# nintendops/DynamicFusion_Body

Measured on AMD Instinct MI355X. Metric: Mvoxels/s TSDF fusion + GN-iters/s warp solve, 256³ grid, 1/2/4/8 GPU, higher is better.
Workload: dtype f64 geometry / f32 volume

## Files before the change

### dynamicfusion_body_amd/csrc/dfh_common.h

```cpp
#pragma once
#include <hip/hip_runtime.h>

#include <cstdarg>
#include <cstdio>

#include "../../include/dfusion_hip.h"

namespace dfh {

char *last_error_buf();
int fail(int code, const char *fmt, ...);

#define DFH_HIP_CHECK(expr)                                                               \
    do {                                                                                  \
        hipError_t _e = (expr);                                                           \
        if (_e != hipSuccess)                                                             \
            return ::dfh::fail(DFH_E_HIP, "%s failed: %s", #expr, hipGetErrorString(_e)); \
    } while (0)

#define DFH_REQUIRE(cond, ...)                                  \
    do {                                                        \
        if (!(cond)) return ::dfh::fail(DFH_E_BADARG, __VA_ARGS__); \
    } while (0)

inline int check_slab(const char *what, const dfh_slab *s) {
    DFH_REQUIRE(s, "%s: null slab", what);
    DFH_REQUIRE(s->res[0] > 0 && s->res[1] > 0 && s->res[2] > 0, "%s: bad grid %dx%dx%d", what, s->res[0], s->res[1], s->res[2]);
    DFH_REQUIRE(0 <= s->x0 && s->x0 <= s->x1 && s->x1 <= s->res[0], "%s: slab [%d,%d) outside [0,%d)", what, s->x0, s->x1, s->res[0]);
    DFH_REQUIRE(s->x1 - s->x0 <= 65535, "%s: slab has more than 65535 planes", what);
    return DFH_OK;
}

inline int check_volume(const char *what, const dfh_volume *v) {
    DFH_REQUIRE(v && v->tsdf && v->tsdf_w, "%s: null volume", what);
    DFH_REQUIRE(v->dtype == DFH_F32 || v->dtype == DFH_F64, "%s: bad volume dtype %d", what, v->dtype);
    return check_slab(what, &v->slab);
}

struct Mat3 { double m[9]; };
struct Mat34 { double m[12]; };
struct Vec3 { double v[3]; };
struct DQ { double q[8]; };

constexpr int kWave = 64;
#ifndef DFH_GN_TILE
#define DFH_GN_TILE 128
#endif
constexpr int kGnTile = DFH_GN_TILE;

#define DFH_OPTION_LIST(X)                                                                                                \
    X(k1_strided) X(k1_late_loads) X(k1_planes_per_block) X(k1_force_scalar) X(k1_bricks_min) X(k1_no_bricks)            \
    X(k1_bricks_nocull) X(k1_no_multi) X(k1_cull) X(k1_nzi) X(k1_prefetch) X(k1_nt) X(k1_gather_first)                  \
    X(k2_exact) X(k2_no_strided) X(k2_nt) X(k3_no_cache) X(k3_exact) X(k3_no_lds) X(k3_wg_per_cu) X(k3_tpb) X(k3_skip) X(plan_radix) X(rigid_atomic) X(gn_reg_own_launch) X(gn_reg_own_gather) \
    X(dbg_gather_part) X(pcg_wpb) X(pcg_multilaunch) X(pcg_spin_limit) X(pcg_one_xcd) X(gn_iter_own_clear) X(gn_gather_full) X(gn_no_view_cull)                                                            \
    X(py_plan_torch) X(py_allreduce_full) X(py_gn_atomic) X(py_gn_no_fused_assoc) X(py_gn_no_fused_iter) X(py_gn_iter_per_call) X(py_no_side_stream) X(py_no_host_scalars)
struct Options {
#define DFH_X(n) long n;
    DFH_OPTION_LIST(DFH_X)
#undef DFH_X
};
const Options &opt();

struct DeviceInfo {
    int n_cu = 0;
    int pcg_occ512 = -1, pcg_occ1024 = -1;
};
DeviceInfo &device_info(int device);
inline bool on(long v) { return v > 0; }

}
```

### dynamicfusion_body_amd/csrc/dfh_plan.hip

```cpp
#include "dfh_common.h"

#include <cstring>

#include <rocprim/device/device_radix_sort.hpp>

namespace dfh {

#ifndef DFH_SORT_BLOCK_ITEMS
#define DFH_SORT_BLOCK_ITEMS 8
#endif
using SortCfg = rocprim::radix_sort_config<rocprim::default_config,
                                           rocprim::merge_sort_config<512, 512, DFH_SORT_BLOCK_ITEMS, 128, 256, 8>,
                                           rocprim::default_config>;
constexpr int kPlanTile = kGnTile;
constexpr int kPlanWaves = kPlanTile / 64;
constexpr int kKMaxP = 8;

__device__ __forceinline__ int plan_find_block(const int *__restrict__ row_ptr, const int *__restrict__ col, int a, int b) {
    int lo = row_ptr[a], hi = row_ptr[a + 1] - 1;
    while (lo <= hi) {
        const int mid = (lo + hi) >> 1;
        const int c = col[mid];
        if (c == b) return mid;
        if (c < b) lo = mid + 1; else hi = mid - 1;
    }
    return -1;
}

__global__ __launch_bounds__(256) void plan_pack_keys_kernel(const int *__restrict__ nbr, int S, int k, unsigned long long N,
                                                              unsigned long long *__restrict__ key, int *__restrict__ idx) {
    const int s = blockIdx.x * 256 + threadIdx.x;
    if (s >= S) return;
    unsigned long long kk = 0;
    for (int j = 0; j < k; ++j) kk = kk * N + (unsigned long long)nbr[(size_t)s * k + j];
    key[s] = kk;
    idx[s] = s;
}

__global__ __launch_bounds__(256) void plan_permute_kernel(const int *__restrict__ order, int S, int k, const double *__restrict__ pos,
                                                           const double *__restrict__ nrm, const int *__restrict__ nbr,
                                                           const double *__restrict__ wts, double *__restrict__ pos_o,
                                                           double *__restrict__ nrm_o, int *__restrict__ nbr_o, double *__restrict__ wts_o) {
    const int i = blockIdx.x * 256 + threadIdx.x;
    if (i >= S) return;
    const size_t src = (size_t)order[i];
#pragma unroll
    for (int c = 0; c < 3; ++c) {
        pos_o[3 * (size_t)i + c] = pos[3 * src + c];
        nrm_o[3 * (size_t)i + c] = nrm[3 * src + c];
    }
    for (int j = 0; j < k; ++j) {
        nbr_o[(size_t)i * k + j] = nbr[src * k + j];
        wts_o[(size_t)i * k + j] = wts[src * k + j];
    }
}

__device__ __forceinline__ bool plan_is_head(const int *__restrict__ nbr, int s, int k) {
    if ((s & (kPlanTile - 1)) == 0) return true;
    bool h = false;
    for (int j = 0; j < k; ++j) h = h || nbr[(size_t)s * k + j] != nbr[(size_t)(s - 1) * k + j];
    return h;
}

__global__ __launch_bounds__(kPlanTile) void plan_heads_kernel(const int *__restrict__ nbr, int S, int k, int *__restrict__ tile_rows) {
    __shared__ int cnt[kPlanWaves];
    const int s = blockIdx.x * kPlanTile + threadIdx.x;
    const bool head = s < S && plan_is_head(nbr, s, k);
    const unsigned long long b = __ballot(head);
    if ((threadIdx.x & 63) == 0) cnt[threadIdx.x >> 6] = __popcll(b);
    __syncthreads();
    if (threadIdx.x == 0) {
        int n = 0;
        for (int w = 0; w < kPlanWaves; ++w) n += cnt[w];
        tile_rows[blockIdx.x] = n;
    }
}

__global__ __launch_bounds__(1024) void plan_scan_kernel(int *__restrict__ tile_rows, int n_tiles, int *__restrict__ n_rows_out) {
    __shared__ int wsum[16];
    __shared__ int carry_s;
    const int lane = threadIdx.x & 63, wv = threadIdx.x >> 6;
    if (threadIdx.x == 0) carry_s = 0;
    __syncthreads();
    for (int base = 0; base < n_tiles; base += 1024) {
        const int i = base + threadIdx.x;
        const int v = i < n_tiles ? tile_rows[i] : 0;
        int x = v;
#pragma unroll
        for (int o = 1; o < 64; o <<= 1) {
            const int y = __shfl_up(x, o, 64);
            if (lane >= o) x += y;
        }
        if (lane == 63) wsum[wv] = x;
        __syncthreads();
        int off = carry_s;
        for (int w = 0; w < wv; ++w) off += wsum[w];
        if (i < n_tiles) tile_rows[i] = off + x - v;
        __syncthreads();
        if (threadIdx.x == 1023) carry_s = off + x;
        __syncthreads();
    }
    if (threadIdx.x == 0) { tile_rows[n_tiles] = carry_s; *n_rows_out = carry_s; }
}

__global__ __launch_bounds__(kPlanTile) void plan_runid_kernel(const int *__restrict__ nbr, int S, int k, const int *__restrict__ tile_off,
                                                          int *__restrict__ run_id, int *__restrict__ row_first) {
    __shared__ int cnt[kPlanWaves];
    const int s = blockIdx.x * kPlanTile + threadIdx.x;
    const int lane = threadIdx.x & 63, wv = threadIdx.x >> 6;
    const bool head = s < S && plan_is_head(nbr, s, k);
    const unsigned long long b = __ballot(head);
    if (lane == 0) cnt[wv] = __popcll(b);
    __syncthreads();
    int r = tile_off[blockIdx.x] + __popcll(b & ((2ull << lane) - 1ull)) - 1;
    for (int w = 0; w < wv; ++w) r += cnt[w];
    if (s < S) {
        run_id[s] = r;
        if (head) row_first[r] = s;
    }
}

__device__ __forceinline__ int plan_count_slot(int *__restrict__ cnt, int key, bool active) {
    const int lane = threadIdx.x & 63;
    unsigned long long todo = __ballot(active);
    int leader = lane, rank = 0, size = 0;
    while (todo) {
        const int l0 = __ffsll((long long)todo) - 1;
        const int k0 = __shfl(key, l0, 64);
        const unsigned long long same = __ballot(active && key == k0) & todo;
        if (active && key == k0) {
            leader = l0;
            rank = __popcll(same & ((1ull << lane) - 1ull));
            size = __popcll(same);
        }
        todo &= ~same;
    }
    int base = 0;
    if (active && leader == lane) base = atomicAdd(cnt + key, size);
    base = __shfl(base, leader, 64);
    return base + rank;
}

__global__ __launch_bounds__(256) void plan_keys_kernel(const int *__restrict__ nbr, const int *__restrict__ row_first, int n_rows, int k,
                                                         const int *__restrict__ row_ptr, const int *__restrict__ col, int B,
                                                         int *__restrict__ blk_key, int *__restrict__ blk_val, int *__restrict__ node_key,
                                                         int *__restrict__ node_val, int *__restrict__ uncovered,
                                                         int *__restrict__ blk_cnt, int *__restrict__ node_cnt) {
    const int row = blockIdx.x * 256 + threadIdx.x;
    const int pr = blockIdx.y, kk = k * k;
    const int sa = pr / k, sb = pr - sa * k;
    const bool in = row < n_rows;
    int blk = B, nb = 0;
    if (in) {
        const size_t s0 = (size_t)row_first[row] * k;
        const int na = nbr[s0 + sa];
        nb = nbr[s0 + sb];
        blk = plan_find_block(row_ptr, col, na, nb);
        if (blk < 0) { blk = B; atomicOr(uncovered, 1); }
    }
    const int slot = plan_count_slot(blk_cnt, blk, in && blk < B);
    if (in) {
        const size_t e = (size_t)row * kk + pr;
        blk_key[e] = blk;
        blk_val[e] = blk < B ? slot : 0;
    }
    if (sa == 0) {
        const int nslot = plan_count_slot(node_cnt, nb, in);
        if (in) {
            node_key[(size_t)row * k + sb] = nb;
            node_val[(size_t)row * k + sb] = nslot;
        }
    }
}

__global__ __launch_bounds__(256) void plan_zero2_kernel(int *__restrict__ a, int na, int *__restrict__ b, int nb) {
    const int i = blockIdx.x * 256 + threadIdx.x;
    if (i < na) a[i] = 0;
    else if (i - na < nb) b[i - na] = 0;
}

__global__ void plan_flag_out_kernel(const int *__restrict__ flag_in, int *__restrict__ flag_out) { *flag_out = *flag_in; }

__global__ __launch_bounds__(1024) void plan_scan2_kernel(int *__restrict__ a, int na, int *__restrict__ b, int nb,
                                                           const int *__restrict__ flag_in, int *__restrict__ flag_out) {
    __shared__ int wsum[16];
    __shared__ int carry_s;
    if (blockIdx.x == 0 && threadIdx.x == 0) *flag_out = *flag_in;
    int *v_ = blockIdx.x == 0 ? a : b;
    const int n = blockIdx.x == 0 ? na : nb;
    const int lane = threadIdx.x & 63, wv = threadIdx.x >> 6;
    if (threadIdx.x == 0) carry_s = 0;
    __syncthreads();
    constexpr int C = 16;
    for (int base = 0; base < n; base += 1024 * C) {
        const int per = min(C, (min(n - base, 1024 * C) + 1023) / 1024);
        const int i0 = base + (int)threadIdx.x * per;
        int v[C];
        int sum = 0;
#pragma unroll
        for (int j = 0; j < C; ++j) {
            v[j] = (j < per && i0 + j < n) ? v_[i0 + j] : 0;
            sum += v[j];
        }
        int x = sum;
#pragma unroll
        for (int o = 1; o < 64; o <<= 1) {
            const int y = __shfl_up(x, o, 64);
            if (lane >= o) x += y;
        }
        if (lane == 63) wsum[wv] = x;
        __syncthreads();
        int off = carry_s;
        for (int w = 0; w < wv; ++w) off += wsum[w];
        int run = off + x - sum;
#pragma unroll
        for (int j = 0; j < C; ++j) {
            if (j < per && i0 + j < n) v_[i0 + j] = run;
            run += v[j];
        }
        __syncthreads();
        if (threadIdx.x == 1023) carry_s = off + x;
        __syncthreads();
    }
    if (threadIdx.x == 0) v_[n] = carry_s;
}

__global__ __launch_bounds__(256) void plan_fill_kernel(const int *__restrict__ blk_key, const int *__restrict__ blk_rank, long E, int B,
                                                         const int *__restrict__ blk_ptr, int *__restrict__ blk_ent,
                                                         const int *__restrict__ node_key, const int *__restrict__ node_rank, long E2,
                                                         const int *__restrict__ node_ptr, int *__restrict__ node_ent) {
    const long e = (long)blockIdx.x * 256 + threadIdx.x;
    if (e < E) {
        const int blk = blk_key[e];
        if (blk < B) blk_ent[blk_ptr[blk] + blk_rank[e]] = (int)e;
    }
    if (e < E2) node_ent[node_ptr[node_key[e]] + node_rank[e]] = (int)e;
}

constexpr int kListLds = 2048;
// ... 217 lines not shown
```

### dynamicfusion_body_amd/csrc/dfh_solve.hip

```cpp
#include "dfh_dq.h"

#include <algorithm>
#include <cmath>
#include <cstring>

namespace dfh {

constexpr int kKMaxS = 8;

struct Q4 { double w, x, y, z; };

__device__ __forceinline__ Q4 qmul(const Q4 &a, const Q4 &b) {
    Q4 o;
    o.w = a.w * b.w - a.x * b.x - a.y * b.y - a.z * b.z;
    o.x = a.w * b.x + a.x * b.w + a.y * b.z - a.z * b.y;
    o.y = a.w * b.y - a.x * b.z + a.y * b.w + a.z * b.x;
    o.z = a.w * b.z + a.x * b.y - a.y * b.x + a.z * b.w;
    return o;
}
__device__ __forceinline__ Q4 qconj(const Q4 &a) { return Q4{a.w, -a.x, -a.y, -a.z}; }
__device__ __forceinline__ Q4 qpure(double x, double y, double z) { return Q4{0.0, x, y, z}; }
__device__ __forceinline__ Q4 qadd(const Q4 &a, const Q4 &b) { return Q4{a.w + b.w, a.x + b.x, a.y + b.y, a.z + b.z}; }
__device__ __forceinline__ Q4 qscale(const Q4 &a, double s) { return Q4{a.w * s, a.x * s, a.y * s, a.z * s}; }

// ... 807 lines not shown
    if (ASSOC && aa.views && aa.cull) {
        __shared__ double sBox[kTileWaves][6];
        __shared__ unsigned sMask;
        const bool in = tid < tile_n;
        double bx[6] = {in ? a_xp.x : __builtin_huge_val(), in ? -a_xp.x : __builtin_huge_val(), in ? a_xp.y : __builtin_huge_val(),
                        in ? -a_xp.y : __builtin_huge_val(), in ? a_xp.z : __builtin_huge_val(), in ? -a_xp.z : __builtin_huge_val()};
#pragma unroll
        for (int o = 32; o > 0; o >>= 1)
#pragma unroll
            for (int c6 = 0; c6 < 6; ++c6) bx[c6] = fmin(bx[c6], __shfl_xor(bx[c6], o, 64));
        if ((tid & 63) == 0)
#pragma unroll
            for (int c6 = 0; c6 < 6; ++c6) sBox[tid >> 6][c6] = bx[c6];
        __syncthreads();
        double box[6];
#pragma unroll
        for (int c6 = 0; c6 < 6; ++c6) {
            double m = sBox[0][c6];
#pragma unroll
            for (int w_ = 1; w_ < kTileWaves; ++w_) m = fmin(m, sBox[w_][c6]);
            box[c6] = (c6 & 1) ? -m : m;
        }
        view_mask = tile_view_mask(aa.ap, aa.views, aa.n_views, box, &sMask);
    }
    if (ASSOC && tid < tile_n)
        a_ok = associate_views<float>(aa.ap, aa.views, aa.n_views, a_xp, a_c, view_mask);
    auto store_assoc = [&]() {
        if (ASSOC && tid < tile_n) {
            corr[3 * (size_t)s] = a_c[0]; corr[3 * (size_t)s + 1] = a_c[1]; corr[3 * (size_t)s + 2] = a_c[2];
            valid[s] = a_ok ? 1 : 0;
        }
    };
    const bool act = ASSOC ? a_ok : (tid < tile_n && valid[s] != 0);
    BT_STAMP(1);
    __shared__ int sWaveCnt[kTileWaves];
    const unsigned long long bal = __ballot(act);
    const int lane = tid & 63, wv = tid >> 6;
    if (lane == 0) sWaveCnt[wv] = __popcll(bal);
    __syncthreads();
    int pos = __popcll(bal & ((1ull << lane) - 1ull));
    for (int w_ = 0; w_ < wv; ++w_) pos += sWaveCnt[w_];
    int n_valid = 0;
#pragma unroll
    for (int w_ = 0; w_ < kTileWaves; ++w_) n_valid += sWaveCnt[w_];
    constexpr int ST_ = gn_row_stride(K);
    double *live = PLANNED ? tile_cost + 2 * (size_t)rt.n_tiles : nullptr;
    const int row_first = PLANNED ? run_id[blockIdx.x * kTile] : 0;
    const int rows_tile = PLANNED ? run_id[blockIdx.x * kTile + tile_n - 1] - row_first + 1 : 0;
    if (n_valid == 0) {
        store_assoc();
        if (PLANNED && tid < rows_tile) live[row_first + tid] = 0.0;
        if (PLANNED && tid == 0) { tile_cost[2 * blockIdx.x] = 0.0; tile_cost[2 * blockIdx.x + 1] = 0.0; }
        return;
    }
    if (!PLANNED && tid == 0) atomicAdd(cost_count + 1, (double)n_valid);
    __shared__ unsigned short sRow[PLANNED ? kTile : 1];
    __shared__ double sObj[kTileWaves];
    double obj = 0.0;
    if (act) {
        if (PLANNED) sRow[pos] = (unsigned short)(run_id[s] - row_first);
        double Jrow[NJ];
        double r;
        if (ASSOC) {
            r = data_row_from(node_dq, idx, w, K, p.lw.q, a_bh, a_nb, a_pf[0], a_pf[1], a_pf[2], a_xp, a_n[0], a_n[1], a_n[2], a_c[0], a_c[1],
                              a_c[2], Jrow);
        } else {
#pragma unroll
            for (int j = 0; j < kKMaxS; ++j) {
                idx[j] = j < K ? nbr[(size_t)s * K + j] : 0;
                w[j] = j < K ? wts[(size_t)s * K + j] : 0.0;
            }
            r = data_row(node_dq, idx, w, K, p.lw.q, spos[3 * (size_t)s], spos[3 * (size_t)s + 1], spos[3 * (size_t)s + 2],
                         snrm[3 * (size_t)s], snrm[3 * (size_t)s + 1], snrm[3 * (size_t)s + 2], corr[3 * (size_t)s],
                         corr[3 * (size_t)s + 1], corr[3 * (size_t)s + 2], Jrow);
        }
        obj = 0.5 * r * r;
        if (p.huber > 0.0 && fabs(r) > p.huber) {
            obj = p.huber * (fabs(r) - 0.5 * p.huber);
            const double sc = sqrt(p.huber / fabs(r));
            r *= sc;
#pragma unroll
            for (int j = 0; j < NJ; ++j) Jrow[j] *= sc;
        }
        if (!PLANNED) {
#pragma unroll
            for (int j = 0; j < K; ++j) sIdx[pos * K + j] = idx[j];
        }
#pragma unroll
        for (int j = 0; j < NJ; ++j) sJ[pos * LD + j] = Jrow[j];
        sJ[pos * LD + NJ] = r;
    }
    store_assoc();
    BT_STAMP(2);
    if (PLANNED) {
#pragma unroll
        for (int o = 32; o > 0; o >>= 1) obj += __shfl_xor(obj, o, 64);
        if (lane == 0) sObj[wv] = obj;
    }
    __syncthreads();
    if (PLANNED && tid == 0) {
        double o = sObj[0];
#pragma unroll
        for (int w_ = 1; w_ < kTileWaves; ++w_) o += sObj[w_];
        tile_cost[2 * blockIdx.x] = o;
        tile_cost[2 * blockIdx.x + 1] = (double)n_valid;
    }
    __shared__ int sRun[kTile + 1];
    __shared__ int sNRuns;
    {
        bool head = false;
        if (tid < n_valid) {
            head = tid == 0;
            if (!head) {
                if (PLANNED) {
                    head = sRow[tid] != sRow[tid - 1];
                } else {
#pragma unroll
                    for (int j = 0; j < K; ++j) head = head || (sIdx[tid * K + j] != sIdx[(tid - 1) * K + j]);
                }
            }
        }
        const unsigned long long hb = __ballot(head);
        if (lane == 0) sWaveCnt[wv] = __popcll(hb);
        __syncthreads();
        int hp = __popcll(hb & ((1ull << lane) - 1ull));
        for (int w_ = 0; w_ < wv; ++w_) hp += sWaveCnt[w_];
        if (head) sRun[hp] = tid;
        if (tid == 0) {
            int n = 0;
            for (int w_ = 0; w_ < kTileWaves; ++w_) n += sWaveCnt[w_];
            sRun[n] = n_valid;
            sNRuns = n;
        }
        __syncthreads();
    }
    const int n_runs = sNRuns;
    BT_STAMP(3);
#ifdef DFH_BUILD_TRACE
    if (threadIdx.x == 0 && blockIdx.x < 8192) g_build_trace[blockIdx.x][6] = (unsigned long long)n_valid | ((unsigned long long)n_runs << 16);
#endif
    constexpr bool kBlkTable = K <= 4 && !PLANNED;
    __shared__ int sBlk[kBlkTable ? kTile * K * K : 1];
    if (kBlkTable) {
        for (int q = tid; q < n_runs * K * K; q += kTile) {
            const int rn = q / (K * K), pr = q - rn * (K * K);
            const int t0 = sRun[rn];
            sBlk[q] = find_block(row_ptr, col, sIdx[t0 * K + pr / K], sIdx[t0 * K + pr % K]);
        }
        __syncthreads();
    }
    constexpr int NUP = PLANNED ? gn_row_gram(K) : NJ * (NJ + 1) / 2;
    if (PLANNED) {
        if (tid < n_runs) partial[(size_t)(row_first + sRow[sRun[tid]]) * ST_ + NUP + NJ + 1] = (double)(sRun[tid + 1] - sRun[tid]);
        __shared__ int sTouched[kTile];
        if (tid < rows_tile) sTouched[tid] = 0;
        __syncthreads();
        if (tid < n_runs) sTouched[sRow[sRun[tid]]] = 1;
        __syncthreads();
        if (tid < rows_tile) live[row_first + tid] = sTouched[tid] ? 1.0 : 0.0;
    }
    BT_STAMP(4);
    if constexpr (PLANNED) {
        constexpr int NC = NJ + 1;
        constexpr int NT = (NC + 15) / 16;
        typedef double d4 __attribute__((ext_vector_type(4)));
        const int li = lane & 15, lk = lane >> 4;
        for (int rn = wv; rn < n_runs; rn += kTile / 64) {
            const int t0 = sRun[rn], t1 = sRun[rn + 1];
            d4 acc[NT * (NT + 1) / 2];
#pragma unroll
            for (int q = 0; q < NT * (NT + 1) / 2; ++q) acc[q] = d4{0.0, 0.0, 0.0, 0.0};
            for (int t = t0; t < t1; t += 4) {
// ... 2237 lines not shown
```

### dynamicfusion_body_amd/solve.py

```python

import ctypes

import numpy as np
import torch

from . import _lib, dist as _dist
from .device import HostScalar, current_stream_ptr, dtype_code, require_gpu


def _f64(a, shape_tail=None):
    t = a if isinstance(a, torch.Tensor) else torch.from_numpy(np.ascontiguousarray(np.asarray(a, dtype=np.float64)))
    t = t.to(device="cuda", dtype=torch.float64).contiguous()
    if shape_tail is not None and tuple(t.shape[1:]) != tuple(shape_tail):
        raise ValueError("array has shape %s, expected (n,%s)" % (tuple(t.shape), ",".join(map(str, shape_tail))))
    return t


def _i32(a, shape_tail=None):
    t = a if isinstance(a, torch.Tensor) else torch.from_numpy(np.ascontiguousarray(np.asarray(a)))
    t = t.to(device="cuda", dtype=torch.int32).contiguous()
    if shape_tail is not None and tuple(t.shape[1:]) != tuple(shape_tail):
        raise ValueError("index array has shape %s, expected (n,%s)" % (tuple(t.shape), ",".join(map(str, shape_tail))))
    return t

# ... 145 lines not shown

    def __init__(self, dev_scalar):
        key = dev_scalar.dtype
        free = _AsyncScalar._pool.setdefault(key, [])
        self._host = free.pop() if free else torch.empty(1, dtype=key).pin_memory()
        self._host.copy_(dev_scalar.reshape(1), non_blocking=True)
        self._event = torch.cuda.Event()
        self._event.record()

    def get(self):
        self._event.synchronize()
        v = int(self._host[0])
        _AsyncScalar._pool[self._host.dtype].append(self._host)
        self._host = None
        return v


def _check_live(live):
    if not (isinstance(live, torch.Tensor) and live.is_cuda and live.dim() == 3 and live.is_contiguous()
            and live.dtype in (torch.float32, torch.float64)):
        raise ValueError("live must be a contiguous 3-D CUDA tensor, float32 or float64")


class WarpSolver:

    def __init__(self, knn=4, pcg_iters=10, distributed=True):
        require_gpu()
        self.lib = _lib.load()
        self.knn = int(knn)
        self.pcg_iters = int(pcg_iters)
        self.distributed = bool(distributed)
        self.force_collective = False
        self.node_nbr = None
        self.S = 0
        self._prob, self._frm, self._sp = _lib.Problem(), _lib.Frame(), _lib.SolveParams()
        self._term = _lib.VolumeTerm()
        if _dist.ranks_share_a_gpu():
            _lib.check(self.lib.dfh_pcg_set_mode(2), "dfh_pcg_set_mode")

    def check_status(self, completed_only=False):
        import ctypes
        n = ctypes.c_long(0)
        fn = self.lib.dfh_pcg_status_peek if completed_only else self.lib.dfh_pcg_status
        rc = fn(current_stream_ptr(), ctypes.byref(n))
        if rc != 0:
            self.lib.dfh_pcg_set_mode(2)
            _lib.check(rc, "dfh_pcg_status")

    def set_graph(self, node_pos, node_dq, node_w, node_nbr=None):
        self.node_pos = _f64(node_pos, (3,))
        self.node_dq = _f64(node_dq, (8,)).clone()
        self.node_w = _f64(node_w, ())
        self.N = self.node_pos.shape[0]
        if not (self.node_dq.shape[0] == self.N == self.node_w.shape[0]):
            raise ValueError("node arrays disagree on the number of nodes")
        self.node_nbr = None if node_nbr is None else _i32(node_nbr, (self.knn,))
        self._pattern = None
        self._pattern_keys = None

    def set_samples(self, pos, nrm, nbr=None, weights=None, sort=True, knn_bricks=None):
        pos, nrm = _f64(pos, (3,)), _f64(nrm, (3,))
        if pos.shape[0] != nrm.shape[0]:
            raise ValueError("sample positions and normals disagree in length")
        if nbr is None:
            nbr, weights = sample_knn(pos, self.node_pos, self.node_w, self.knn, bricks=knn_bricks)
        else:
            nbr = _i32(nbr, (self.knn,))
            if weights is None:
                d = pos[:, None, :] - self.node_pos[nbr.long()]
                dist = torch.sqrt((d[..., 0] * d[..., 0] + d[..., 1] * d[..., 1]) + d[..., 2] * d[..., 2])
                weights = torch.exp(-1.0 * (dist / (2 * self.node_w[nbr.long()])) ** 2)
            weights = _f64(weights, (self.knn,))
        self.order = None
        self._tuple_key = None
        if sort and pos.shape[0] > 0:
            if float(self.N) ** self.knn < 2.0 ** 62 and not _lib.opt_on("py_plan_torch"):
                pos, nrm, nbr, weights = self._sort_samples_device(pos, nrm, nbr, weights)
            else:
                key = self._pack_tuples(nbr)
                if key is not None:
                    key, self.order = torch.sort(key, stable=True)
                    self._tuple_key = key
                else:
                    _, inv = torch.unique(nbr, dim=0, return_inverse=True)
                    self.order = torch.argsort(inv, stable=True)
                pos, nrm, nbr, weights = self._permute(pos, nrm, nbr, weights)
        self.spos, self.snrm = pos.contiguous(), nrm.contiguous()
        self.snbr, self.swts = nbr.contiguous(), weights.contiguous()
        self.S = pos.shape[0]
        self.corr = torch.empty((self.S, 3), dtype=torch.float64, device="cuda")
        self.valid = torch.zeros(self.S, dtype=torch.uint8, device="cuda")
        self._pattern = None

    def _sort_samples_device(self, pos, nrm, nbr, weights):
        S = pos.shape[0]
        pos, nrm, nbr, weights = pos.contiguous(), nrm.contiguous(), nbr.contiguous(), weights.contiguous()
        out = (torch.empty_like(pos), torch.empty_like(nrm), torch.empty_like(nbr), torch.empty_like(weights))
        key = torch.empty(S, dtype=torch.int64, device="cuda")
        order = torch.empty(S, dtype=torch.int32, device="cuda")
        nbytes = self.lib.dfh_gn_sort_workspace_bytes(S)
        ws = torch.empty((nbytes + 7) // 8, dtype=torch.int64, device="cuda")
        _lib.check(self.lib.dfh_gn_sort_samples(pos.data_ptr(), nrm.data_ptr(), nbr.data_ptr(), weights.data_ptr(), S, self.knn, self.N,
                                                out[0].data_ptr(), out[1].data_ptr(), out[2].data_ptr(), out[3].data_ptr(), key.data_ptr(),
                                                order.data_ptr(), ws.data_ptr(), ws.numel() * 8, current_stream_ptr()), "dfh_gn_sort_samples")
        self._tuple_key = key
        self._order32 = order
        self.order = _LazyLong(order)
        return out

    def _permute(self, pos, nrm, nbr, weights):
        pos, nrm, nbr, weights = pos.contiguous(), nrm.contiguous(), nbr.contiguous(), weights.contiguous()
        out = (torch.empty_like(pos), torch.empty_like(nrm), torch.empty_like(nbr), torch.empty_like(weights))
        order = self.order.contiguous()
        _lib.check(self.lib.dfh_permute_samples(order.data_ptr(), pos.shape[0], self.knn, pos.data_ptr(), nrm.data_ptr(), nbr.data_ptr(),
                                                weights.data_ptr(), out[0].data_ptr(), out[1].data_ptr(), out[2].data_ptr(),
                                                out[3].data_ptr(), current_stream_ptr()), "dfh_permute_samples")
        return out

    def _pack_tuples(self, nbr):
        if float(self.N) ** self.knn >= 2.0 ** 62:
            return None
        key = nbr[:, 0].long()
        for j in range(1, self.knn):
            key = key * self.N + nbr[:, j].long()
        return key

    def _unpack_tuples(self, key):
        cols = []
        for _ in range(self.knn):
            cols.append(key % self.N)
            key = key // self.N
        return torch.stack(cols[::-1], dim=1)

    def prepare(self, overlap=()):
        if self._pattern is None:
            self._build_pattern(overlap)

    def _build_pattern(self, overlap=()):
        N, k = self.N, self.knn
        new = []
        old = getattr(self, "_pattern_keys", None)
        if old is not None:
            nbytes = self.lib.dfh_pcg_workspace_bytes(N, self.pcg_iters)
            if self.pcg_ws.numel() * 8 < nbytes:
                self.pcg_ws = torch.empty((nbytes + 7) // 8, dtype=torch.float64, device="cuda")
            covered = self._build_plan(old, reg=False, overlap=overlap)
            if (_dist.all_ranks(covered) if self.distributed else covered):
                self._pattern = True
                return
            if self.S > 0:
                new.append(self._pair_keys_of_rows())
            new.append(old)
        elif self.S > 0:
            if self._tuple_key is not None:
                tup = self._unpack_tuples(torch.unique_consecutive(self._tuple_key))
            else:
                tup = torch.unique(self.snbr, dim=0).long()
            new.append((tup[:, :, None] * N + tup[:, None, :]).reshape(-1))
        if old is None:
            new.append(torch.arange(N, device="cuda", dtype=torch.int64) * (N + 1))
            if self.node_nbr is not None:
                i = torch.arange(N, device="cuda", dtype=torch.int64)[:, None].expand(N, k)
                j = self.node_nbr.long()
                new += [(i * N + j).reshape(-1), (j * N + i).reshape(-1)]
        if self.S > 0 and N <= 4096 and old is not None:
            pk = new[0]
            pi, pj = pk // N, pk % N
            lim = ((self.node_pos[pi] - self.node_pos[pj]) ** 2).sum(dim=1).max() * (1.15 * 1.15)
            dd = ((self.node_pos[:, None, :] - self.node_pos[None, :, :]) ** 2).sum(dim=2)
            near = torch.nonzero(dd <= lim)
            new.append(near[:, 0] * N + near[:, 1])
        keys = torch.cat(new)
        keys = _dist.union_sorted_keys(keys) if self.distributed else torch.unique(keys)
        self._pattern_keys = keys
        rows = (keys // N).to(torch.int32)
        self.col = (keys % N).to(torch.int32).contiguous()
        self.row_ptr = torch.searchsorted(rows.contiguous(), torch.arange(N + 1, device="cuda", dtype=torch.int32)).to(torch.int32).contiguous()
        self.B = int(keys.numel())
        self.system = torch.zeros(self.B * 36 + 6 * N + 2, dtype=torch.float64, device="cuda")
        self.vals = self.system[:self.B * 36]
        self.rhs = self.system[self.B * 36:self.B * 36 + 6 * N]
        self.cost_count = self.system[self.B * 36 + 6 * N:]
        upper_m = self.col >= rows
        mkey_s = self.col.to(torch.int64) * N + rows.to(torch.int64)
        mirror_s = torch.searchsorted(keys, mkey_s).clamp(max=self.B - 1)
        self.blk_upper, self.n_upper = None, 0
        if bool((keys[mirror_s] == mkey_s).all()):
            ids = torch.nonzero(upper_m).flatten()
            mir = torch.where(self.col[ids] == rows[ids], torch.full_like(ids, -1), mirror_s[ids])
            self.blk_upper = torch.stack([ids, mir], dim=1).to(torch.int32).contiguous()
            self.n_upper = int(ids.numel())
        self._tri = None
        if self.distributed and (_dist.world()[1] > 1 or self.force_collective) and not _lib.opt_on("py_allreduce_full"):
            upper = self.col >= rows
            up_rank = (torch.cumsum(upper.to(torch.int64), 0) - 1)
            mkey = self.col.to(torch.int64) * N + rows.to(torch.int64)
            mirror = torch.searchsorted(keys, mkey).clamp(max=self.B - 1)
            if bool((keys[mirror] == mkey).all()):
                src = torch.where(upper, up_rank, up_rank[mirror]).to(torch.int32).contiguous()
                n_upper = int(upper.sum())
                self._tri = (rows.contiguous(), src, n_upper, torch.empty(36 * n_upper + 6 * N + 2, dtype=torch.float64, device="cuda"))
        self.dx = torch.empty(6 * N, dtype=torch.float64, device="cuda")
        nbytes = self.lib.dfh_pcg_workspace_bytes(N, self.pcg_iters)
        self.pcg_ws = torch.empty((nbytes + 7) // 8, dtype=torch.float64, device="cuda")
        self._build_plan(keys)
        self._pattern = True

    def _build_plan(self, keys, reg=True, overlap=()):
        if self.S == 0 or self._tuple_key is None or _lib.opt_on("py_plan_torch"):
            return self._build_plan_torch(keys, reg)
        N, k, S, dev = self.N, self.knn, self.S, "cuda"
        tile = int(self.lib.dfh_gn_tile_samples())
        n_tiles = (S + tile - 1) // tile
        tile_off = torch.empty(n_tiles + 1, dtype=torch.int32, device=dev)
        n_rows_d = None if HostScalar.enabled else torch.empty(1, dtype=torch.int32, device=dev)
        pending = HostScalar(torch.int32) if HostScalar.enabled else None
        _lib.check(self.lib.dfh_gn_plan_count(self.snbr.data_ptr(), S, k, tile_off.data_ptr(),
                                              pending.ptr() if pending is not None else n_rows_d.data_ptr(), current_stream_ptr()),
                   "dfh_gn_plan_count")
        if pending is None:
            pending = _AsyncScalar(n_rows_d)
        if len(overlap) > 0:
            overlap[0]()
        R = pending.get()
        self.n_rows = R
        if R * k * k >= 2 ** 31:
            raise ValueError("too many sample runs for 32-bit plan entries")
        self.run_id = torch.empty(S, dtype=torch.int32, device=dev)
        self._row_first = torch.empty(R, dtype=torch.int32, device=dev)
        self.blk_ptr = torch.empty(self.B + 1, dtype=torch.int32, device=dev)
        self.blk_ent = torch.empty(R * k * k, dtype=torch.int32, device=dev)
        self.node_ptr = torch.empty(N + 1, dtype=torch.int32, device=dev)
        self.node_ent = torch.empty(R * k, dtype=torch.int32, device=dev)
        unc_h = HostScalar(torch.int32) if HostScalar.enabled and not reg else None
        unc = torch.empty(1, dtype=torch.int32, device=dev) if unc_h is None else None
        nbytes = self.lib.dfh_gn_plan_workspace_bytes(R, k)
        ws = torch.empty((nbytes + 7) // 8, dtype=torch.int64, device=dev)
        _lib.check(self.lib.dfh_gn_plan_build(self.snbr.data_ptr(), S, k, N, tile_off.data_ptr(), R, self.row_ptr.data_ptr(),
                                              self.col.data_ptr(), self.B, self.run_id.data_ptr(), self._row_first.data_ptr(),
                                              self.blk_ptr.data_ptr(), self.blk_ent.data_ptr(), self.node_ptr.data_ptr(),
                                              self.node_ent.data_ptr(), unc.data_ptr() if unc_h is None else unc_h.ptr(), ws.data_ptr(), ws.numel() * 8,
                                              current_stream_ptr()), "dfh_gn_plan_build")
        ne = int(self.lib.dfh_gn_partial_doubles(k))
        self.partial = torch.empty(max(1, R * ne) + 2 * n_tiles + R, dtype=torch.float64, device=dev)
        self._pair_keys = None
        if reg:
            self._build_reg_plan(keys)
            return True
        pending = _AsyncScalar(unc) if unc_h is None else unc_h
        if len(overlap) > 1:
            overlap[1]()
        return pending.get() == 0

    def _pair_keys_of_rows(self):
        if getattr(self, "_pair_keys", None) is None:
            tup = self.snbr[self._row_first.long()].long()
            self._pair_keys = (tup[:, :, None] * self.N + tup[:, None, :]).reshape(-1)
        return self._pair_keys

    def _csr_lists(self, tup, keys):
        N, dev = self.N, "cuda"
        i32 = lambda t: t.to(torch.int32).contiguous()
        key = (tup[:, :, None] * N + tup[:, None, :]).reshape(-1)
        blk = torch.searchsorted(keys, key)
        covered = (keys[blk.clamp(max=keys.numel() - 1)] == key).all()
        sblk, order = torch.sort(blk.to(torch.int32), stable=True)
        bp = torch.searchsorted(sblk, torch.arange(self.B + 1, device=dev, dtype=torch.int32), out_int32=True)
        snode, order2 = torch.sort(tup.reshape(-1).to(torch.int32), stable=True)
        npt = torch.searchsorted(snode, torch.arange(N + 1, device=dev, dtype=torch.int32), out_int32=True)
        return (bp, i32(order), npt, i32(order2)), key, covered

    def _build_reg_plan(self, keys):
        N, k, dev = self.N, self.knn, "cuda"
        self.partial_reg = None
        if self.node_nbr is not None:
            ii = torch.arange(N, device=dev, dtype=torch.int64)[:, None].expand(N, k).reshape(-1)
            pair = torch.stack([ii, self.node_nbr.long().reshape(-1)], dim=1)
            (self.rblk_ptr, self.rblk_ent, self.rnode_ptr, self.rnode_ent), _, _ = self._csr_lists(pair, keys)
            self.partial_reg = torch.zeros(N * k * int(self.lib.dfh_gn_partial_doubles(2)), dtype=torch.float64, device=dev)

    def _build_plan_torch(self, keys, reg=True):
        N, k, S, dev = self.N, self.knn, self.S, "cuda"
        if S == 0:
            self.run_id = torch.zeros(1, dtype=torch.int32, device=dev)
            self.n_rows = 0
            tup = torch.zeros((0, k), dtype=torch.int64, device=dev)
            self._row_first = torch.zeros(0, dtype=torch.int32, device=dev)
        else:
            head = torch.empty(S, dtype=torch.bool, device=dev)
            head[1:] = (self._tuple_key[1:] != self._tuple_key[:-1]) if self._tuple_key is not None else \
                (self.snbr[1:] != self.snbr[:-1]).any(dim=1)
            head[::int(self.lib.dfh_gn_tile_samples())] = True
            self.run_id = torch.cumsum(head, 0, dtype=torch.int32).sub_(1)
            self._row_first = torch.nonzero(head).reshape(-1).to(torch.int32)
            tup = self.snbr[head].long()
            self.n_rows = int(tup.shape[0])
        R = self.n_rows
        (self.blk_ptr, self.blk_ent, self.node_ptr, self.node_ent), self._pair_keys, covered = self._csr_lists(tup, keys)
        if reg:
            self._build_reg_plan(keys)
        ne = int(self.lib.dfh_gn_partial_doubles(k))
        tile = int(self.lib.dfh_gn_tile_samples())
        self.partial = torch.empty(max(1, R * ne) + 2 * ((S + tile - 1) // tile) + R, dtype=torch.float64, device=dev)
        if R * k * k >= 2 ** 31:
            raise ValueError("too many sample runs for 32-bit plan entries")
        return bool(covered) if not reg else True

    def _order_index(self):
        return self.order.long() if isinstance(self.order, _LazyLong) else self.order

    def set_correspondences(self, corr, valid=None):
        c = _f64(corr, (3,))
        if c.shape[0] != self.S:
            raise ValueError("Please first call setupCorrespondences to compute point to point correspondences "
                             "between canonical and live frame vertices!")
        self.corr = c[self._order_index()].contiguous() if self.order is not None else c
        if valid is None:
            self.valid = torch.ones(self.S, dtype=torch.uint8, device="cuda")
        else:
            v = valid if isinstance(valid, torch.Tensor) else torch.from_numpy(np.asarray(valid))
            v = v.to(device="cuda", dtype=torch.uint8)
            self.valid = v[self._order_index()].contiguous() if self.order is not None else v.contiguous()

    _PROBLEM_TENSORS = (("sample_pos", "spos"), ("sample_nrm", "snrm"), ("nbr", "snbr"), ("weights", "swts"), ("corr", "corr"),
                        ("valid", "valid"), ("node_dq", "node_dq"), ("node_pos", "node_pos"), ("node_w", "node_w"),
                        ("row_ptr", "row_ptr"), ("col", "col"), ("vals", "vals"), ("rhs", "rhs"), ("cost_count", "cost_count"),
                        ("blk_upper", "blk_upper"), ("run_id", "run_id"), ("partial", "partial"), ("blk_ptr", "blk_ptr"),
                        ("blk_ent", "blk_ent"), ("node_ptr", "node_ptr"), ("node_ent", "node_ent"), ("partial_reg", "partial_reg"),
                        ("rblk_ptr", "rblk_ptr"), ("rblk_ent", "rblk_ent"), ("rnode_ptr", "rnode_ptr"), ("rnode_ent", "rnode_ent"))

    def _problem(self, lw_dq, rw=0.0, huber=0.0, reg=True, plan=True, upper=True):
        p = self._prob
        for field, attr in self._PROBLEM_TENSORS:
            t = getattr(self, attr, None)
            setattr(p, field, 0 if t is None else t.data_ptr())
        p.n_samples, p.knn, p.n_nodes = self.S, self.knn, self.N
        p.node_nbr = self.node_nbr.data_ptr() if (reg and self.node_nbr is not None and rw != 0.0) else 0
        p.lw_dq, p.rw, p.huber_delta = _lib.darr(lw_dq, 8), float(rw), float(huber)
        p.n_blocks, p.n_rows = getattr(self, "B", 0), getattr(self, "n_rows", 0)
        p.n_upper = self.n_upper if upper and p.blk_upper else 0
        if not upper:
            p.blk_upper = 0
        if not plan:
            p.blk_ptr = 0
        return p

    @staticmethod
    def _views(depth, lw_cam):
        if isinstance(depth, (list, tuple)):
            depths, lws = list(depth), list(lw_cam)
            if len(depths) != len(lws) or not depths:
                raise ValueError('length of camera matrix array must equal that of depth maps')
            return depths, lws
        return [depth], [lw_cam]

    def _views_table(self, depths, lw_cams):
        for d in depths:
            if not (isinstance(d, torch.Tensor) and d.is_cuda and d.dim() == 2 and d.is_contiguous()):
                raise ValueError("depth must be a contiguous 2-D CUDA tensor")
            if d.shape != depths[0].shape or d.dtype != depths[0].dtype:
                raise ValueError("the depth maps of one frame must share a shape and a dtype")
        n = len(depths)
        lw = np.ascontiguousarray(np.stack([np.asarray(m, dtype=np.float64).reshape(12) for m in lw_cams]))
        key = (tuple(int(d.data_ptr()) for d in depths), tuple(int(d._version) for d in depths), lw.tobytes(), current_stream_ptr())
        if getattr(self, "_views_key", None) != key:
            ptrs = (ctypes.c_void_p * n)(*[int(d.data_ptr()) for d in depths])
            Hh, Ww = (int(v) for v in depths[0].shape)
            dt = dtype_code(depths[0])
            buf = torch.empty(self.lib.dfh_gn_views_bytes(n, dt, Hh, Ww), dtype=torch.uint8, device="cuda")
            _lib.check(self.lib.dfh_gn_pack_views(buf.data_ptr(), n, ptrs, dt, Hh, Ww, lw.ctypes.data_as(ctypes.POINTER(ctypes.c_double)),
                                                  current_stream_ptr()), "dfh_gn_pack_views")
            self._views_key, self._views_buf, self._views_keep = key, buf, list(depths)
        H, W = depths[0].shape
        return self._views_buf, n, int(H), int(W)

    def _frame(self, depth, lw_cam, K, Kinv, scale, center, half, max_dist):
        depths, lws = self._views(depth, lw_cam)
        tab, n, H, W = self._views_table(depths, lws)
# ... 193 lines not shown
```

Baseline: 501,800.

## Canonicalize neighbor tuples by sorting node indices so permuted sets share plan rows

Sample neighbor tuples are reduced to a canonical sorted order before they are keyed, grouped into runs and turned into block-pair lists, in both the HIP plan kernels and the torch fallback. The Jacobian columns in the solve kernel are scattered to match the canonical slots. Samples whose neighbor sets differ only in order then merge into the same run, which means fewer rows, fewer partial sums and fewer distinct block pairs in the Gauss-Newton assembly. In exchange, every sample pays a small O(k²) ranking step and the plan kernels gain an LDS staging pass and a barrier.

```diff
diff --git a/dynamicfusion_body_amd/csrc/dfh_common.h b/dynamicfusion_body_amd/csrc/dfh_common.h
--- a/dynamicfusion_body_amd/csrc/dfh_common.h
+++ b/dynamicfusion_body_amd/csrc/dfh_common.h
@@ -48,6 +48,18 @@
 #endif
 constexpr int kGnTile = DFH_GN_TILE;
 
+template <int KM>
+__device__ __forceinline__ void canonical_slots(const int (&idx)[KM], int k, int (&canon)[KM]) {
+#pragma unroll
+    for (int j = 0; j < KM; ++j) {
+        int c = 0;
+#pragma unroll
+        for (int m = 0; m < KM; ++m)
+            if (m != j && m < k) c += (idx[m] < idx[j] || (m < j && idx[m] == idx[j])) ? 1 : 0;
+        canon[j] = c;
+    }
+}
+
 #define DFH_OPTION_LIST(X)                                                                                                \
     X(k1_strided) X(k1_late_loads) X(k1_planes_per_block) X(k1_force_scalar) X(k1_bricks_min) X(k1_no_bricks)            \
     X(k1_bricks_nocull) X(k1_no_multi) X(k1_cull) X(k1_nzi) X(k1_prefetch) X(k1_nt) X(k1_gather_first)                  \
diff --git a/dynamicfusion_body_amd/csrc/dfh_plan.hip b/dynamicfusion_body_amd/csrc/dfh_plan.hip
--- a/dynamicfusion_body_amd/csrc/dfh_plan.hip
+++ b/dynamicfusion_body_amd/csrc/dfh_plan.hip
@@ -27,12 +27,31 @@
     return -1;
 }
 
+__device__ __forceinline__ void plan_canonical_tuple(const int *__restrict__ nbr, size_t s, int k, int (&ct)[kKMaxP]) {
+    int idx[kKMaxP], canon[kKMaxP];
+#pragma unroll
+    for (int j = 0; j < kKMaxP; ++j) idx[j] = j < k ? nbr[s * k + j] : 0;
+    canonical_slots(idx, k, canon);
+#pragma unroll
+    for (int p = 0; p < kKMaxP; ++p) {
+        int v = 0;
+#pragma unroll
+        for (int j = 0; j < kKMaxP; ++j)
+            if (j < k && canon[j] == p) v = idx[j];
+        ct[p] = v;
+    }
+}
+
 __global__ __launch_bounds__(256) void plan_pack_keys_kernel(const int *__restrict__ nbr, int S, int k, unsigned long long N,
                                                               unsigned long long *__restrict__ key, int *__restrict__ idx) {
     const int s = blockIdx.x * 256 + threadIdx.x;
     if (s >= S) return;
+    int ct[kKMaxP];
+    plan_canonical_tuple(nbr, (size_t)s, k, ct);
     unsigned long long kk = 0;
-    for (int j = 0; j < k; ++j) kk = kk * N + (unsigned long long)nbr[(size_t)s * k + j];
+#pragma unroll
+    for (int j = 0; j < kKMaxP; ++j)
+        if (j < k) kk = kk * N + (unsigned long long)ct[j];
     key[s] = kk;
     idx[s] = s;
 }
@@ -55,17 +74,30 @@
     }
 }
 
-__device__ __forceinline__ bool plan_is_head(const int *__restrict__ nbr, int s, int k) {
-    if ((s & (kPlanTile - 1)) == 0) return true;
+__device__ __forceinline__ bool plan_is_head(const int *__restrict__ nbr, int s, int S, int k, int (&sct)[kKMaxP][kPlanTile]) {
+    const int t = threadIdx.x;
+    int ct[kKMaxP];
+    if (s < S) {
+        plan_canonical_tuple(nbr, (size_t)s, k, ct);
+#pragma unroll
+        for (int p = 0; p < kKMaxP; ++p)
+            if (p < k) sct[p][t] = ct[p];
+    }
+    __syncthreads();
+    if (s >= S) return false;
+    if (t == 0) return true;
     bool h = false;
-    for (int j = 0; j < k; ++j) h = h || nbr[(size_t)s * k + j] != nbr[(size_t)(s - 1) * k + j];
+#pragma unroll
+    for (int p = 0; p < kKMaxP; ++p)
+        if (p < k) h = h || ct[p] != sct[p][t - 1];
     return h;
 }
 
 __global__ __launch_bounds__(kPlanTile) void plan_heads_kernel(const int *__restrict__ nbr, int S, int k, int *__restrict__ tile_rows) {
     __shared__ int cnt[kPlanWaves];
+    __shared__ int sct[kKMaxP][kPlanTile];
     const int s = blockIdx.x * kPlanTile + threadIdx.x;
-    const bool head = s < S && plan_is_head(nbr, s, k);
+    const bool head = plan_is_head(nbr, s, S, k, sct);
     const unsigned long long b = __ballot(head);
     if ((threadIdx.x & 63) == 0) cnt[threadIdx.x >> 6] = __popcll(b);
     __syncthreads();
@@ -106,9 +138,10 @@
 __global__ __launch_bounds__(kPlanTile) void plan_runid_kernel(const int *__restrict__ nbr, int S, int k, const int *__restrict__ tile_off,
                                                           int *__restrict__ run_id, int *__restrict__ row_first) {
     __shared__ int cnt[kPlanWaves];
+    __shared__ int sct[kKMaxP][kPlanTile];
     const int s = blockIdx.x * kPlanTile + threadIdx.x;
     const int lane = threadIdx.x & 63, wv = threadIdx.x >> 6;
-    const bool head = s < S && plan_is_head(nbr, s, k);
+    const bool head = plan_is_head(nbr, s, S, k, sct);
     const unsigned long long b = __ballot(head);
     if (lane == 0) cnt[wv] = __popcll(b);
     __syncthreads();
@@ -152,9 +185,14 @@
     const bool in = row < n_rows;
     int blk = B, nb = 0;
     if (in) {
-        const size_t s0 = (size_t)row_first[row] * k;
-        const int na = nbr[s0 + sa];
-        nb = nbr[s0 + sb];
+        int ct[kKMaxP];
+        plan_canonical_tuple(nbr, (size_t)row_first[row], k, ct);
+        int na = 0;
+#pragma unroll
+        for (int p = 0; p < kKMaxP; ++p) {
+            if (p == sa) na = ct[p];
+            if (p == sb) nb = ct[p];
+        }
         blk = plan_find_block(row_ptr, col, na, nb);
         if (blk < 0) { blk = B; atomicOr(uncovered, 1); }
     }
diff --git a/dynamicfusion_body_amd/csrc/dfh_solve.hip b/dynamicfusion_body_amd/csrc/dfh_solve.hip
--- a/dynamicfusion_body_amd/csrc/dfh_solve.hip
+++ b/dynamicfusion_body_amd/csrc/dfh_solve.hip
@@ -913,12 +913,16 @@
 #pragma unroll
             for (int j = 0; j < NJ; ++j) Jrow[j] *= sc;
         }
+        int canon[kKMaxS];
+        canonical_slots(idx, K, canon);
         if (!PLANNED) {
 #pragma unroll
-            for (int j = 0; j < K; ++j) sIdx[pos * K + j] = idx[j];
-        }
-#pragma unroll
-        for (int j = 0; j < NJ; ++j) sJ[pos * LD + j] = Jrow[j];
+            for (int j = 0; j < K; ++j) sIdx[pos * K + canon[j]] = idx[j];
+        }
+#pragma unroll
+        for (int j = 0; j < K; ++j)
+#pragma unroll
+            for (int i = 0; i < 6; ++i) sJ[pos * LD + 6 * canon[j] + i] = Jrow[6 * j + i];
         sJ[pos * LD + NJ] = r;
     }
     store_assoc();
diff --git a/dynamicfusion_body_amd/solve.py b/dynamicfusion_body_amd/solve.py
--- a/dynamicfusion_body_amd/solve.py
+++ b/dynamicfusion_body_amd/solve.py
@@ -251,7 +251,7 @@
                     key, self.order = torch.sort(key, stable=True)
                     self._tuple_key = key
                 else:
-                    _, inv = torch.unique(nbr, dim=0, return_inverse=True)
+                    _, inv = torch.unique(self._canonical(nbr), dim=0, return_inverse=True)
                     self.order = torch.argsort(inv, stable=True)
                 pos, nrm, nbr, weights = self._permute(pos, nrm, nbr, weights)
         self.spos, self.snrm = pos.contiguous(), nrm.contiguous()
@@ -286,9 +286,14 @@
                                                 out[3].data_ptr(), current_stream_ptr()), "dfh_permute_samples")
         return out
 
+    @staticmethod
+    def _canonical(nbr):
+        return torch.sort(nbr, dim=1, stable=True).values
+
     def _pack_tuples(self, nbr):
         if float(self.N) ** self.knn >= 2.0 ** 62:
             return None
+        nbr = self._canonical(nbr)
         key = nbr[:, 0].long()
         for j in range(1, self.knn):
             key = key * self.N + nbr[:, j].long()
@@ -324,7 +329,7 @@
             if self._tuple_key is not None:
                 tup = self._unpack_tuples(torch.unique_consecutive(self._tuple_key))
             else:
-                tup = torch.unique(self.snbr, dim=0).long()
+                tup = torch.unique(self._canonical(self.snbr), dim=0).long()
             new.append((tup[:, :, None] * N + tup[:, None, :]).reshape(-1))
         if old is None:
             new.append(torch.arange(N, device="cuda", dtype=torch.int64) * (N + 1))
@@ -423,7 +428,7 @@
 
     def _pair_keys_of_rows(self):
         if getattr(self, "_pair_keys", None) is None:
-            tup = self.snbr[self._row_first.long()].long()
+            tup = self._canonical(self.snbr[self._row_first.long()]).long()
             self._pair_keys = (tup[:, :, None] * self.N + tup[:, None, :]).reshape(-1)
         return self._pair_keys
 
@@ -457,12 +462,13 @@
             self._row_first = torch.zeros(0, dtype=torch.int32, device=dev)
         else:
             head = torch.empty(S, dtype=torch.bool, device=dev)
+            canon = self._canonical(self.snbr)
             head[1:] = (self._tuple_key[1:] != self._tuple_key[:-1]) if self._tuple_key is not None else \
-                (self.snbr[1:] != self.snbr[:-1]).any(dim=1)
+                (canon[1:] != canon[:-1]).any(dim=1)
             head[::int(self.lib.dfh_gn_tile_samples())] = True
             self.run_id = torch.cumsum(head, 0, dtype=torch.int32).sub_(1)
             self._row_first = torch.nonzero(head).reshape(-1).to(torch.int32)
-            tup = self.snbr[head].long()
+            tup = canon[head].long()
             self.n_rows = int(tup.shape[0])
         R = self.n_rows
         (self.blk_ptr, self.blk_ent, self.node_ptr, self.node_ent), self._pair_keys, covered = self._csr_lists(tup, keys)
```

After: 497,700. About the same (-0.8%).
